# WanqingXia/UR-gym

Measured on AMD Instinct MI355X. Metric: env-steps/sec (whole node), higher is better.
Workload: dtype f64; 1 GPU; UR5DynReach-v1 N=65536 per GPU, random actions U(-1,1), auto-reset, seed 0; envs_total=65536, gather_obs=False, rollout_api=False, gjk_start=bullet

## Files before the change

### ur_gym_amd/csrc/urgym_device.h

```cpp
#pragma once
#include <stdint.h>
#if defined(URGYM_HOST_HARNESS)
#include <cmath>
#define __device__
#define __forceinline__ inline
#define URGYM_LDS
static inline uint32_t __umulhi(uint32_t a, uint32_t b) { return (uint32_t)(((uint64_t)a * b) >> 32); }
using std::fma; using std::sqrt; using std::fabs; using std::fmin; using std::fmax; using std::acos; using std::asin; using std::atan2;
#else
#include <hip/hip_runtime.h>
#define URGYM_LDS __attribute__((address_space(3)))
#endif
#include "urgym_philox.h"

namespace urgym {

struct D3 {
  double x, y, z;
};
__device__ __forceinline__ D3 d3(double x, double y, double z) { return D3{x, y, z}; }
__device__ __forceinline__ D3 operator+(D3 a, D3 b) { return d3(a.x + b.x, a.y + b.y, a.z + b.z); }
__device__ __forceinline__ D3 operator-(D3 a, D3 b) { return d3(a.x - b.x, a.y - b.y, a.z - b.z); }
__device__ __forceinline__ D3 operator-(D3 a) { return d3(-a.x, -a.y, -a.z); }
__device__ __forceinline__ D3 operator*(D3 a, double s) { return d3(a.x * s, a.y * s, a.z * s); }
// ... 253 lines not shown
  if (d3_ >= 0.0 && d4 <= d3_) { mask = 2; return b; }
  double vc = d1 * d4 - d3_ * d2;
  if (vc <= 0.0 && d1 >= 0.0 && d3_ <= 0.0) { mask = 3; return a + ab * (d1 / (d1 - d3_)); }
  double d5 = -dot(ab, c), d6 = -dot(ac, c);
  if (d6 >= 0.0 && d5 <= d6) { mask = 4; return c; }
  double vb = d5 * d2 - d1 * d6;
  if (vb <= 0.0 && d2 >= 0.0 && d6 <= 0.0) { mask = 5; return a + ac * (d2 / (d2 - d6)); }
  double va = d3_ * d6 - d5 * d4;
  if (va <= 0.0 && (d4 - d3_) >= 0.0 && (d5 - d6) >= 0.0) {
    mask = 6;
    return b + (c - b) * ((d4 - d3_) / ((d4 - d3_) + (d5 - d6)));
  }
  double den = 1.0 / (va + vb + vc);
  mask = 7;
  return a + ab * (vb * den) + ac * (vc * den);
}

enum { GJK_PENETRATING = 1, GJK_ITERCAP = 2, GJK_SEPARATED = 4, GJK_CLOSE = 8  };

constexpr int GJK_SLOT_DOUBLES = 24;
__device__ __forceinline__ D3 ldw(XRef T, int i) { return d3(T.at(12 + 3 * i), T.at(13 + 3 * i), T.at(14 + 3 * i)); }
__device__ __forceinline__ void stw(XRef T, int i, D3 w) { T.set(12 + 3 * i, w.x); T.set(13 + 3 * i, w.y); T.set(14 + 3 * i, w.z); }

struct GjkRun {
  D3 v;
  double sq;
  int n;
  int iter;
  int info;
  double core;
  bool done;
};
__device__ __forceinline__ void gjk_begin(GjkRun& r, D3 v0) {
  r.v = v0;
  r.sq = 1.0e300;
  r.n = 0;
  r.iter = 0;
  r.info = 0;
  r.core = 0.0;
  r.done = false;
}
__device__ __forceinline__ void gjk_finish(GjkRun& r, bool check_simplex, bool separated) {
  const double REL_ERROR2 = 1.0e-12;
  const double l2 = len2(r.v);
  r.done = true;
  if (!check_simplex || l2 < REL_ERROR2) {
    if (!(r.info & GJK_ITERCAP)) r.info |= GJK_PENETRATING;
    r.core = 0.0;
    return;
  }
  if (separated) r.info |= GJK_SEPARATED;
  r.core = sqrt(l2);
}
__device__ __forceinline__ void gjk_iterate(GjkRun& r, const HullMap& g, const ShapeDesc& A, XRef T, const ShapeDesc& B, double max_d,
                                            double verdict_d = 0.0) {
  const double REL_ERROR2 = 1.0e-12;
  const double EPS = 2.220446049250313e-16;
  const D3 W0 = ldw(T, 0), W1 = ldw(T, 1), W2 = ldw(T, 2);
  D3 w;
  {
    X3 TX;
#pragma unroll
    for (int k = 0; k < 9; k++) TX.r[k] = T.at(k);
    TX.t = d3(T.at(9), T.at(10), T.at(11));
    const D3 dA = rotT(TX, -r.v);
    int rec = 0;
    if (A.type == SH_HULL) rec = g.cell[A.hull * DIRMAP_CELLS + dirmap_cell(dA)];
    const D3 q = support_local(g, B, r.v);
    const D3 sA = (A.type == SH_HULL) ? hull_support_from(g, rec, dA) : support_local(g, A, dA);
    const D3 p = apply(TX, sA);
    w = p - q;
  }
  int fin = 0;
  const double delta = dot(r.v, w);
  if (delta > 0.0 && delta * delta > r.sq * (max_d * max_d)) fin = 1 | 4;
  if (fin == 0) {
    const bool in = (((int)(r.n > 0) & (int)(len2(W0 - w) <= 1e-12)) | ((int)(r.n > 1) & (int)(len2(W1 - w) <= 1e-12)) |
                     ((int)(r.n > 2) & (int)(len2(W2 - w) <= 1e-12))) != 0;
    const double f0 = r.sq - delta, f1 = r.sq * REL_ERROR2;
    if (in || f0 <= f1) fin = 1;
  }
  if (fin == 0) {
    stw(T, r.n, w);
    int n = r.n + 1;
    D3 nv = d3(0, 0, 0);
    bool valid = true;
    int used = 15;
    bool reduce = true;
    if (n == 1) {
      nv = w;
      reduce = false;
    } else if (n == 2) {
      D3 s0 = W0;
      D3 e = w - s0;
      double t = -dot(e, s0);
      used = 3;
      if (t > 0.0) {
        double ee = dot(e, e);
        if (t < ee) t /= ee;
        else { t = 1.0; used = 2; }
      } else {
        t = 0.0;
        used = 1;
      }
      nv = s0 + e * t;
    } else {
      const bool tetra = (n == 4);
      auto face_vertices = [](int f, int& ia, int& ib, int& ic, int& io) {
        ia = (f == 3) ? 1 : 0;
        ib = (f == 0) ? 1 : ((f == 1) ? 2 : 3);
        ic = (f == 0) ? 2 : ((f == 1) ? 3 : ((f == 2) ? 1 : 2));
        io = (f == 0) ? 3 : ((f == 1) ? 1 : ((f == 2) ? 2 : 0));
      };
      int todo = 1;
      bool degen = false;
      if (tetra) {
        todo = 0;
        auto plane = [&](D3 a, D3 b, D3 c, D3 o, int bit) {
          const D3 nrm = cross(b - a, c - a);
          const double signp = -dot(a, nrm), signd = dot(o - a, nrm);
          if (signd * signd < (1.0e-8 * 1.0e-8)) degen = true;
// ... 6 lines not shown
      }
      double best = 1.0e300;
      used = -1;
#pragma unroll 1
      while (todo) {
        const int f = __builtin_ctz((unsigned)todo);
        todo &= todo - 1;
        int ia, ib, ic, io;
        face_vertices(f, ia, ib, ic, io);
        const D3 a = ldw(T, ia), b = ldw(T, ib), c = ldw(T, ic);
        int m3;
        const D3 pt = tri_closest(a, b, c, m3);
        const double l = len2(pt);
        if (used < 0 || l < best) {
          best = l;
          nv = pt;
          used = ((m3 & 1) ? (1 << ia) : 0) | ((m3 & 2) ? (1 << ib) : 0) | ((m3 & 4) ? (1 << ic) : 0);
        }
      }
      if (degen) {
        valid = false;
        reduce = false;
      } else if (used < 0) {
        nv = d3(0, 0, 0);
        reduce = false;
      }
    }
    if (reduce) {
      if (n >= 4 && !(used & 8)) { n--; }
      if (n >= 3 && !(used & 4)) { n--; stw(T, 2, ldw(T, n)); }
      if (n >= 2 && !(used & 2)) { n--; stw(T, 1, ldw(T, n)); }
      if (n >= 1 && !(used & 1)) { n--; stw(T, 0, ldw(T, n)); }
    }
    r.n = n;
    if (!valid) fin = 1;
    else {
      const double nsq = len2(nv);
      if (nsq < REL_ERROR2) { r.v = nv; fin = 1; }
      else if (nsq <= verdict_d * verdict_d) { r.v = nv; r.info |= GJK_CLOSE; fin = 1; }
      else {
        const double prev = r.sq;
        r.sq = nsq;
        if (prev - nsq <= EPS * prev) fin = 1;
        else {
          r.v = nv;
          if (r.iter++ > 1000) { r.info |= GJK_ITERCAP; fin = 3; }
          else if (n == 4) fin = 3;
        }
      }
    }
  }
  if (fin) gjk_finish(r, !(fin & 2), (fin & 4) != 0);
}


constexpr int EPA_MAX_VERTS = 48, EPA_MAX_FACES = 128;
constexpr int EPA_FACE_GROUPS = EPA_MAX_FACES / 64;
constexpr double EPA_TOL = 1.0e-9, EPA_CAP_RESIDUAL = 1.0e-5;
#if !defined(URGYM_HOST_HARNESS)
struct EpaWs {
  URGYM_LDS double* base;
  int stride;
  __device__ __forceinline__ URGYM_LDS double* at(int r, int c) const { return base + r * stride + c; }
  __device__ __forceinline__ D3 point(int v) const {
    const int r = 3 * (v / 63), c = 1 + v % 63;
    return d3(*at(r, c), *at(r + 1, c), *at(r + 2, c));
  }
  __device__ __forceinline__ void set_point(int v, D3 p) const {
    const int r = 3 * (v / 63), c = 1 + v % 63;
    *at(r, c) = p.x; *at(r + 1, c) = p.y; *at(r + 2, c) = p.z;
  }
  __device__ __forceinline__ URGYM_LDS int* face_word(int f) const {
    return f < 126 ? (URGYM_LDS int*)at(6, 1) + f : (URGYM_LDS int*)at(7, 1) + (f - 126);
  }
  __device__ __forceinline__ URGYM_LDS unsigned short* rim(int c) const { return (URGYM_LDS unsigned short*)at(8 + c / 252, 1) + c % 252; }
  __device__ __forceinline__ URGYM_LDS unsigned char* free_slot(int r) const { return (URGYM_LDS unsigned char*)at(11, 1) + r; }
  __device__ __forceinline__ URGYM_LDS double* plane(int f, int k) const { return at(12 + 4 * (f >> 6) + k, f & 63); }
};
__device__ __forceinline__ void epa_wave_sync() {
  __builtin_amdgcn_fence(__ATOMIC_ACQ_REL, "wavefront");
  __builtin_amdgcn_wave_barrier();
}
__device__ __forceinline__ bool epa_plane(D3 pi, D3 pj, D3 pk, D3& n, double& d) {
  const D3 c = cross(pj - pi, pk - pi);
  const double l2 = len2(c);
  if (l2 > 1e-40) {
    n = c * (1.0 / sqrt(l2));
    d = dot(n, pi);
    return true;
  }
  n = d3(0, 0, 0);
  d = 1e300;
  return false;
}
__device__ inline double epa_wave(const HullMap& g, const ShapeDesc& A, const ShapeDesc& B, EpaWs ws, int lane, bool& capped) {
  const XRef T{ws.base, ws.stride};
  auto supp = [&](D3 n) -> D3 { return apply(T, support_local(g, A, rotT(T, n))) - support_local(g, B, -n); };
  const double t = 0.5773502691896258;
  {
    const D3 p0 = supp(d3(t, t, t)), p1 = supp(d3(t, -t, -t)), p2 = supp(d3(-t, t, -t)), p3 = supp(d3(-t, -t, t));
    if (lane == 0) { ws.set_point(0, p0); ws.set_point(1, p1); ws.set_point(2, p2); ws.set_point(3, p3); }
#pragma unroll
    for (int gi = 0; gi < EPA_FACE_GROUPS; gi++) *ws.face_word(lane + 64 * gi) = 0;
    epa_wave_sync();
    if (lane < 4) {
      int i = lane == 3 ? 1 : 0, j = lane == 0 ? 1 : (lane == 1 ? 3 : (lane == 2 ? 2 : 3)), k = lane == 0 ? 2 : (lane == 1 ? 1 : (lane == 2 ? 3 : 2));
// ... 132 lines not shown
```

### ur_gym_amd/csrc/urgym_hip.hip

```cpp
#include <hip/hip_runtime.h>
#include <stdint.h>
#include <stdio.h>
#include <string.h>
#include <math.h>
#include <new>
#include <vector>

#include "../../include/urgym.h"
#include "../../data/ur5e_model.h"
#include "urgym_device.h"
#include "urgym_launch_plan.h"
#include "urgym_actor.h"
#include "urgym_critic.h"
#include "urgym_pack_map.h"
#include "urgym_weights.h"
#include "urgym_replay.h"
#include "urgym_tables_host.h"

using namespace urgym;


namespace {

constexpr int WAVES = 4;
constexpr int THREADS = GROUP * WAVES;
constexpr uint32_t NO_ITEM = 0xFFFFFFFFu;
constexpr int REFILL_MIN = 16;
constexpr int RESIDENT = 3;
constexpr int SC_ROWS = 19;
constexpr int PAIR_TABLE = 0, PAIR_TRACK = 5, PAIR_SELF = 10;
__host__ __device__ constexpr int self_pair_bit(int la, int lb) {
  return PAIR_SELF + (la == 1 ? 0 : (la == 2 ? 4 : 7)) + (lb - (la + 2));
}

enum { MODE_STEP = 0, MODE_RESET = 1, MODE_REFRESH = 2, MODE_PREFETCH = 3 };
enum { Q_TABLE = 0, Q_TRACK = 1, Q_SELF = 2 };

constexpr double M_HULL = 0.001, M_PRIM = 0.001;
constexpr double CYL_R = 0.05, CYL_H = 0.4, M_CYL = M_PRIM;
constexpr double TABLE_CX = 0.5, TABLE_CY = 0.0, TABLE_CZ = -0.58, TABLE_HX = 0.55, TABLE_HY = 0.9, TABLE_HZ = 0.46;
constexpr double M_TABLE = M_PRIM;
constexpr double TRACK_CX = 0.0, TRACK_CY = 0.0, TRACK_CZ = -0.06, TRACK_HX = 0.1, TRACK_HY = 0.55, TRACK_HZ = 0.06;
constexpr double M_TRACK = M_PRIM;
constexpr double TARGET_BOX_H = 0.025, M_TARGET_BOX = M_PRIM, TARGET_SPHERE_R = 0.02;

struct DevTables {
  double joint_rot[6][9];
  double joint_xyz[6][3];
  double capsule[6][7];
};
__constant__ DevTables c_tab;

constexpr int REC_FIELDS = 36;
enum { REC_GOAL = 0, REC_START = 6, REC_END = 12, REC_VEL = 18, REC_QUAT = 24, REC_LD = 28, REC_DP = 33 };

struct KParams {
  urgym_config cfg;
  urgym_buffers buf;
  HullMap graph;
  int obs_dim, goal_dim;
  uint32_t seed_lo, seed_hi;
  int pp;
  int copy_final;
  int envs;
  int big_blocks;
  int envs_tail;
  double* rec_d;
  int32_t* rec_i;
  int2* rlist;
  int* rcount;
  int rcap;
  double* ld_scratch;
  double* sc_scratch;
  int* rzero;
  int* rzero2;
  int fallback_on;
  int prefetch;
  int inline_ori;
  float neutral_ach[6];
};
__device__ __forceinline__ double& REC(const KParams& P, int slot, int f, int n) {
  return P.rec_d[((size_t)slot * REC_FIELDS + f) * P.cfg.num_envs + n];
}
__device__ __forceinline__ int32_t& RECI(const KParams& P, int slot, int j, int n) {
  return P.rec_i[((size_t)slot * 2 + j) * P.cfg.num_envs + n];
}

__device__ __forceinline__ double& SOA(double* base, int f, int n, int N) { return base[(size_t)f * N + n]; }

__device__ __forceinline__ long long sortable(double x) {
  const long long k = __double_as_longlong(x);
  return k ^ ((k >> 63) & 0x7FFFFFFFFFFFFFFFLL);
}
__device__ __forceinline__ double unsortable(long long k) { return __longlong_as_double(k ^ ((k >> 63) & 0x7FFFFFFFFFFFFFFFLL)); }

__device__ __forceinline__ ShapeDesc hull_desc(int link ) {
  ShapeDesc s;
  s.type = SH_HULL; s.hull = link - 1; s.hx = s.hy = s.hz = 0.0;
  return s;
}
__device__ __forceinline__ ShapeDesc cyl_desc() {
  ShapeDesc s;
  s.type = SH_CYLZ; s.hull = 0;
  s.hx = s.hy = CYL_R - M_CYL; s.hz = 0.5 * CYL_H - M_CYL;
  return s;
}
__device__ __forceinline__ ShapeDesc box_desc(double hx, double hy, double hz, double margin) {
  ShapeDesc s;
  s.type = SH_BOX; s.hull = 0;
  s.hx = hx - margin; s.hy = hy - margin; s.hz = hz - margin;
  return s;
}
__device__ __forceinline__ ShapeDesc point_desc() {
  ShapeDesc s;
  s.type = SH_POINT; s.hull = 0; s.hx = s.hy = s.hz = 0.0;
  return s;
}

__device__ __forceinline__ void fk_joint(X3& T, int k, double s, double c) {
  const double* F = c_tab.joint_rot[k];
  const double* o = c_tab.joint_xyz[k];
  T.t = T.t + rot(T, d3(o[0], o[1], o[2]));
  double g[9];
#pragma unroll
  for (int i = 0; i < 3; i++) {
    g[i * 3 + 0] = F[i * 3 + 0] * c + F[i * 3 + 1] * s;
    g[i * 3 + 1] = F[i * 3 + 1] * c - F[i * 3 + 0] * s;
    g[i * 3 + 2] = F[i * 3 + 2];
  }
  double r[9];
#pragma unroll
// ... 458 lines not shown
          if (seg_box_lower_bound(b0, b1, TABLE_CX, TABLE_CY, TABLE_CZ, TABLE_HX, TABLE_HY, TABLE_HZ) - rb <= lim) pairs |= 1u << (PAIR_TABLE + link - 2);
          if (seg_box_lower_bound(b0, b1, TRACK_CX, TRACK_CY, TRACK_CZ, TRACK_HX, TRACK_HY, TRACK_HZ) - rb <= lim) pairs |= 1u << (PAIR_TRACK + link - 2);
        }
#pragma unroll
        for (int A = 1; A <= 3; A++) {
          if (A <= link - 2) {
            if (segseg_dist(a0[A - 1], a1[A - 1], b0, b1) - c_tab.capsule[A - 1][6] - rb <= lim + M_HULL) pairs |= 1u << self_pair_bit(A, link);
          }
        }
      }
      if (MODE == MODE_STEP) {
        double er, ep, ey;
        rpy_from_quat(rot_to_quat(T.r), er, ep, ey);
        float* orow = B.observation + (size_t)n * OD;
        orow[0] = (float)T.t.x; orow[1] = (float)T.t.y; orow[2] = (float)T.t.z;
        orow[3] = (float)er; orow[4] = (float)ep; orow[5] = (float)ey;
        atomicOr(&s_flags[e], EE_BIT);
      }
    }
    s_pairs[e] = pairs;
    if (pairs) atomicAdd(&s_pending, __popc(pairs));
  }
  if (MODE == MODE_STEP) {
    if (wv >= WAVES - G && lane == 0) __hip_atomic_fetch_add(&s_p1done, 1, __ATOMIC_RELEASE, __HIP_MEMORY_SCOPE_WORKGROUP);
  } else {
    __syncthreads();
  }

  if (!(MODE == MODE_STEP && !HAS_OBST && !cfg.check_collision)) {
    D3 v0 = d3(0, 1, 0);
    int kind = 3, e = 0, lb = 2, la = 1;
    auto shape_a = [&]() -> ShapeDesc { return hull_desc(kind == Q_SELF ? la : lb); };
    auto shape_b = [&]() -> ShapeDesc {
      ShapeDesc s;
      s.type = (kind == 3) ? SH_CYLZ : ((kind == Q_SELF) ? SH_HULL : SH_BOX);
      s.hull = lb - 1;
      const bool tbl = (kind == Q_TABLE);
      s.hx = (kind == 3) ? (CYL_R - M_CYL) : (tbl ? (TABLE_HX - M_TABLE) : (TRACK_HX - M_TRACK));
      s.hy = (kind == 3) ? (CYL_R - M_CYL) : (tbl ? (TABLE_HY - M_TABLE) : (TRACK_HY - M_TRACK));
      s.hz = (kind == 3) ? (0.5 * CYL_H - M_CYL) : (tbl ? (TABLE_HZ - M_TABLE) : (TRACK_HZ - M_TRACK));
      return s;
    };
    bool exact = false;
    const bool guided = cfg.gjk_start == URGYM_GJK_START_GUIDED;
    auto capsule_mid = [&](int link, const X3& TX) -> D3 {
      const double* c = c_tab.capsule[link - 1];
      return apply(TX, d3(0.5 * (c[0] + c[3]), 0.5 * (c[1] + c[4]), 0.5 * (c[2] + c[5])));
    };
    auto guided_axis = [&](D3 mid, D3 centre) -> D3 {
      const D3 d = mid - centre;
      const double n2 = dot(d, d);
      return n2 > 1e-12 ? d * (1.0 / sqrt(n2)) : d3(0, 1, 0);
    };
    bool p1_ok = false;
    auto setup = [&](uint32_t item) -> bool {
      e = item & 255;
      kind = (item >> 8) & 3;
      exact = ((item >> 16) & 1) != 0;
      lb = (item >> 10) & 7;
      la = (item >> 13) & 7;
      if (e >= E || lb < 1 || lb > 6 || (kind == Q_SELF && (la < 1 || la > 6))) return false;
      const int n = s_env[e];
      if (n < 0) return false;
      const bool cached = (MODE == MODE_STEP) && p1_ok;
      if (MODE == MODE_STEP && !cached) {
        bool finite = true;
        for (int k = 0; k < 6; k++) finite = finite && (fabs(joint_of_step<MODE>(P, actions, n, k)) < 1.0e6);
        if (!finite) return false;
      }
      X3 T = identity_x3(), TA = identity_x3();
#pragma unroll 1
      for (int k = 0; k < lb; k++) {
        double sn, cs;
        if (cached) { sn = SOA(P.sc_scratch, 2 * k, n, N); cs = SOA(P.sc_scratch, 2 * k + 1, n, N); }
        else sincos(LDS_Q ? s_q[k][e] : joint_of_step<MODE>(P, actions, n, k), &sn, &cs);
        fk_joint(T, k, sn, cs);
        if (k + 1 == la) TA = T;
      }
      if (kind == 3) {
        X3 To;
        if (LDS_STATE) {
          quat_to_rot(Q4{s_obst[3][e], s_obst[4][e], s_obst[5][e], s_obst[6][e]}, To.r);
          To.t = d3(s_obst[0][e], s_obst[1][e], s_obst[2][e]);
        } else if (cached) {
          quat_to_rot(Q4{SOA(P.sc_scratch, 15, n, N), SOA(P.sc_scratch, 16, n, N), SOA(P.sc_scratch, 17, n, N), SOA(P.sc_scratch, 18, n, N)}, To.r);
          To.t = d3(SOA(P.sc_scratch, 12, n, N), SOA(P.sc_scratch, 13, n, N), SOA(P.sc_scratch, 14, n, N));
        } else {
          double op[3];
          Q4 oqs;
          obstacle_of_step<KIND>(P, n, op, oqs);
          quat_to_rot(oqs, To.r);
          To.t = d3(op[0], op[1], op[2]);
        }
        store(pose_slot, rel(To, T));
        v0 = rotT(To, guided ? guided_axis(capsule_mid(lb, T), To.t) : d3(0, 1, 0));
      } else if (kind == Q_SELF) {
        store(pose_slot, rel(T, TA));
        v0 = rotT(T, guided ? guided_axis(capsule_mid(la, TA), capsule_mid(lb, T)) : d3(0, 1, 0));
      } else {
        const bool tbl = (kind == Q_TABLE);
        const D3 centre = d3(tbl ? TABLE_CX : TRACK_CX, tbl ? TABLE_CY : TRACK_CY, tbl ? TABLE_CZ : TRACK_CZ);
        v0 = guided ? guided_axis(capsule_mid(lb, T), centre) : d3(0, 1, 0);
        T.t = T.t - centre;
        store(pose_slot, T);
      }
      return true;
    };
    auto claim_pair = [&]() -> uint32_t {
      int pe = tid % E;
#pragma unroll 1
      for (int trip = 0; trip < 2 * ME; trip++, pe = (pe + 1 == E ? 0 : pe + 1)) {
        uint32_t m = s_pairs[pe];
        while (m) {
          const int b = __ffs((int)m) - 1;
          const uint32_t old = atomicAnd(&s_pairs[pe], ~(1u << b));
          if (old & (1u << b)) {
            if (b < PAIR_TRACK) return (uint32_t)pe | (Q_TABLE << 8) | ((uint32_t)(b - PAIR_TABLE + 2) << 10);
            if (b < PAIR_SELF) return (uint32_t)pe | (Q_TRACK << 8) | ((uint32_t)(b - PAIR_TRACK + 2) << 10);
            const int i = b - PAIR_SELF;
            const int la = i < 4 ? 1 : (i < 7 ? 2 : 3);
            const int l2 = i < 4 ? 3 + i : (i < 7 ? i : i - 2);
            return (uint32_t)pe | (Q_SELF << 8) | ((uint32_t)l2 << 10) | ((uint32_t)la << 13);
          }
          m = old & ~(1u << b);
        }
      }
      return NO_ITEM;
    };
    auto margin_sum = [&]() -> double {
      return M_HULL + ((kind == 3) ? M_CYL : ((kind == Q_SELF) ? M_HULL : ((kind == Q_TABLE) ? M_TABLE : M_TRACK)));
    };
    const int n_tickets = HAS_OBST ? (workbench ? 15 : 5) * E : 0;
    auto ticket_item = [&](int t) -> uint32_t {
      const int body = t / (5 * E), r = t - body * 5 * E;
      const int tl = r / E, te = r - tl * E, link = 2 + tl;
      if (body == 0) return (uint32_t)te | (3u << 8) | ((uint32_t)link << 10);
      return (uint32_t)te | ((uint32_t)(body == 1 ? Q_TABLE : Q_TRACK) << 8) | ((uint32_t)link << 10) | (1u << 16);
    };

    GjkRun run;
    bool busy = false;
    if (MODE == MODE_STEP) p1_ok = __hip_atomic_load(&s_p1done, __ATOMIC_ACQUIRE, __HIP_MEMORY_SCOPE_WORKGROUP) >= G;
    if (tid < n_tickets) {
      busy = setup(ticket_item(tid));
      if (busy) gjk_begin(run, v0);
    }
    for (;;) {
      if (busy) {
        if (MODE == MODE_STEP) {
          const URGYM_LDS double* row = (const URGYM_LDS double*)(URGYM_LDS void*)&L.s_kind[kind | ((int)exact << 2)][0];
          ShapeDesc sb;
          sb.type = (kind == 3) ? SH_CYLZ : ((kind == Q_SELF) ? SH_HULL : SH_BOX);
          sb.hull = lb - 1;
          sb.hx = row[0]; sb.hy = row[1]; sb.hz = row[2];
          gjk_iterate(run, P.graph, shape_a(), pose_slot, sb, row[3], row[4]);
        } else {
          const bool wants_distance = (kind == 3 || exact);
          const double verdict_d = wants_distance ? 0.0 : margin_sum() + cfg.collision_margin;
          gjk_iterate(run, P.graph, shape_a(), pose_slot, shape_b(), wants_distance ? margin_sum() + 0.02 + 5.0 : verdict_d, verdict_d);
        }
        if (run.done) {
          const double msum = margin_sum();
          if (kind == 3 || exact) {
            double dist = run.core - msum;
            if (run.info & GJK_PENETRATING) {
              dist = -msum;
              const int body = (kind == 3) ? 0 : (kind == Q_TABLE ? 1 : 2);
              atomicOr(&s_flags[e], URGYM_STATUS_PENETRATION | (need_epa ? (1 << (EPA_SHIFT + 5 * body + (lb - 2))) : 0));
            }
            if (run.info & GJK_ITERCAP) atomicOr(&s_flags[e], URGYM_STATUS_GJK_ITER);
            if (workbench) atomicMin(reinterpret_cast<long long*>(dist_cell(lb - 2, e)), sortable(dist));
            else *dist_cell(lb - 2, e) = dist;
          } else {
            const bool hit = (run.info & (GJK_PENETRATING | GJK_CLOSE)) || (!(run.info & GJK_SEPARATED) && (run.core - msum) <= cfg.collision_margin);
            if (hit) atomicOr(&s_flags[e], COLL_BIT);
          }
          busy = false;
        }
      }
      typedef int pool_words __attribute__((ext_vector_type(4)));
      const pool_words pool = *(volatile URGYM_LDS pool_words*)(URGYM_LDS void*)&s_ticket;
      __builtin_amdgcn_fence(__ATOMIC_ACQUIRE, "workgroup");
      const bool more_tickets = pool.x < n_tickets;
      const bool p1_published = (MODE != MODE_STEP) || pool.z >= G;
      const bool more_pairs = pool.y > 0;
      if (MODE == MODE_STEP) p1_ok = p1_published;
      const int idle_lanes = __popcll(__ballot(!busy));
      if (!busy && (idle_lanes >= REFILL_MIN || idle_lanes == 64)) {
        uint32_t item = NO_ITEM;
        if (more_tickets) {
          const int t = atomicAdd(&s_ticket, 1);
          if (t < n_tickets) item = ticket_item(t);
        } else if (more_pairs) {
          if (atomicSub(&s_pending, 1) > 0) item = claim_pair();
        }
        if (item != NO_ITEM) {
          busy = setup(item);
          if (busy) gjk_begin(run, v0);
        }
      }
      if (__ballot(busy) == 0ull && !more_tickets && !more_pairs && p1_published) break;
    }
    auto epa_pass = [&]() -> bool {
      const EpaWs ws{(URGYM_LDS double*)&s_pose[0][0] + GROUP * wv, THREADS};
      bool armed = false;
#pragma unroll 1
      for (int g = 0; g < G; g++) {
        const int sl = g * GROUP + lane;
        const int marks = (sl < E) ? ((__hip_atomic_load(&s_flags[sl], __ATOMIC_RELAXED, __HIP_MEMORY_SCOPE_WORKGROUP) & EPA_MASK) >> EPA_SHIFT) : 0;
        unsigned long long envs_marked = __ballot(marks != 0);
#pragma unroll 1
        while (envs_marked) {
          const int el = __builtin_ctzll(envs_marked);
          envs_marked &= envs_marked - 1ull;
          const int ee = g * GROUP + el;
          int me = __shfl(marks, el);
#pragma unroll 1
          while (me) {
            const int b = __builtin_ctz((unsigned)me);
            me &= me - 1;
            int mine = 0;
            if (lane == 0) mine = (atomicAnd(&s_flags[ee], ~(1 << (EPA_SHIFT + b))) >> (EPA_SHIFT + b)) & 1;
            if (!__shfl(mine, 0)) continue;
            if (!armed) {
              pose_slot.p = ws.base;
              if (MODE == MODE_STEP) p1_ok = true;
              armed = true;
            }
            const int body = b / 5, link = 2 + b - 5 * body;
            const uint32_t item = (uint32_t)ee | ((uint32_t)(body == 0 ? 3 : (body == 1 ? Q_TABLE : Q_TRACK)) << 8) | ((uint32_t)link << 10) |
                                  ((body ? 1u : 0u) << 16);
            if (!setup(item)) continue;
            epa_wave_sync();
            bool capped;
            const double depth = epa_wave(P.graph, shape_a(), shape_b(), ws, lane, capped);
            if (lane == 0) {
              const double dist = -(depth + margin_sum());
              if (workbench) atomicMin(reinterpret_cast<long long*>(dist_cell(lb - 2, e)), sortable(dist));
              else *dist_cell(lb - 2, e) = dist;
              if (capped) atomicOr(&s_flags[e], URGYM_STATUS_GJK_ITER);
            }
          }
        }
      }
      if (armed) pose_slot.p = (URGYM_LDS double*)&s_pose[0][0] + tid;
      return armed;
    };
    if (HAS_OBST && WITH_EPA) {
      if (lane == 0) __hip_atomic_fetch_add(&s_left, 1, __ATOMIC_RELEASE, __HIP_MEMORY_SCOPE_WORKGROUP);
#pragma unroll 1
      for (;;) {
        const int left = __hip_atomic_load(&s_left, __ATOMIC_ACQUIRE, __HIP_MEMORY_SCOPE_WORKGROUP);
        const bool served = epa_pass();
        if (!served && left >= WAVES) break;
        if (!served) __builtin_amdgcn_s_sleep(16);
      }
    }
    __syncthreads();
  }

  const int pe = (wv - (WAVES - G)) * GROUP + lane;
  if (wv >= WAVES - G && pe < E && s_env[pe] != -1) {
    const int n = s_env[pe] >= 0 ? s_env[pe] : -2 - s_env[pe];
    double q[6];
    for (int i = 0; i < 6; i++) q[i] = LDS_Q ? s_q[i][pe] : joint_of_step<MODE>(P, actions, n, i);
    const bool ee_ready = (MODE == MODE_STEP) && (s_flags[pe] & EE_BIT);
    X3 TE = identity_x3();
    if (!ee_ready) {
      if (KIND == URGYM_ENV_ORI) {
        double sn[6], cs[6];
#pragma unroll
        for (int k = 0; k < 6; k++) sincos(q[k], &sn[k], &cs[k]);
#pragma unroll
        for (int k = 0; k < 6; k++) fk_joint(TE, k, sn[k], cs[k]);
      } else {
#pragma unroll 1
        for (int k = 0; k < 6; k++) {
          double sn, cs;
          sincos(q[k], &sn, &cs);
          fk_joint(TE, k, sn, cs);
        }
      }
    }
    double opos[3] = {0, 0, 0};
    Q4 oq{0, 0, 0, 1};
// ... 509 lines not shown
  c->near_threshold = 0.2;
  c->collision_margin = 0.01;
  c->target_clearance = 0.1;
  c->min_travel = 1.0;
  c->dyn_time_duration = 2.0;
  const double neutral[6] = {0.0, -1.5708, 0.0, -1.5708, 0.0, 0.0};
  for (int i = 0; i < 6; i++) c->neutral_q[i] = neutral[i];
  if (env_kind == URGYM_ENV_ORI) {
    c->w_distance = -70; c->w_orientation = -30;
    const double gl[3] = {0.3, -0.5, 0.0}, gh[3] = {0.75, 0.5, 0.2};
    for (int i = 0; i < 3; i++) { c->goal_low[i] = gl[i]; c->goal_high[i] = gh[i]; }
  } else if (env_kind == URGYM_ENV_OBS) {
    c->w_distance = -100; c->w_orientation = 0;
    const double gl[3] = {0.3, -0.5, -0.1}, gh[3] = {0.75, 0.5, 0.2}, ol[3] = {0.5, -0.5, 0.25}, oh[3] = {1.0, 0.5, 0.55};
    for (int i = 0; i < 3; i++) { c->goal_low[i] = gl[i]; c->goal_high[i] = gh[i]; c->obst_low[i] = ol[i]; c->obst_high[i] = oh[i]; }
    for (int i = 0; i < 5; i++) c->w_link[i] = 100.0;
  } else {
    c->w_distance = -70; c->w_orientation = -30;
    const double gl[3] = {0.4, -0.5, 0.0}, gh[3] = {0.75, 0.5, 0.2}, ol[3] = {0.5, -0.8, 0.25}, oh[3] = {1.2, 0.8, 0.75};
    const double sgl[3] = {0.3, -0.5, 0.0}, sgh[3] = {0.75, 0.5, 0.2}, sol[3] = {0.5, -0.5, 0.25}, soh[3] = {1.0, 0.5, 0.55};
    const bool sta = env_kind == URGYM_ENV_STA;
    for (int i = 0; i < 3; i++) {
      c->goal_low[i] = sta ? sgl[i] : gl[i]; c->goal_high[i] = sta ? sgh[i] : gh[i];
      c->obst_low[i] = sta ? sol[i] : ol[i]; c->obst_high[i] = sta ? soh[i] : oh[i];
    }
    const double lw[5] = {8, 2.4, 1.2, 1.2, 0.2};
    double sum = 0;
    for (int i = 0; i < 5; i++) sum += lw[i];
    for (int i = 0; i < 5; i++) c->w_link[i] = lw[i] / sum * 50;
  }
}

KParams make_params(Handle* h, int copy_final) {
  KParams P{};
  P.cfg = h->cfg;
  P.buf = h->buf;
  P.graph.recs = h->d_recs;
  P.graph.cell = h->d_cell;
  P.obs_dim = h->obs_dim;
  P.goal_dim = h->goal_dim;
  P.seed_lo = (uint32_t)h->seed;
  P.seed_hi = (uint32_t)(h->seed >> 32);
  P.pp = h->pp;
  P.copy_final = copy_final;
  P.envs = h->plan.step_envs;
  P.big_blocks = h->plan.big_blocks;
  P.envs_tail = h->plan.tail_envs;
  P.rec_d = h->d_rec;
  P.rec_i = h->d_reci;
  P.ld_scratch = h->d_ld_scratch;
  P.sc_scratch = h->d_sc_scratch;
  P.fallback_on = 1;
  P.inline_ori = h->plan.inline_ori ? 1 : 0;
  for (int i = 0; i < 6; i++) P.neutral_ach[i] = h->neutral_ach[i];
  return P;
}

template <int MODE>
void launch_mode(Handle* h, KParams P, const float* actions, hipStream_t s, int envs = 0, long items = -1) {
  long blocks = h->plan.step_blocks;
  if (MODE != MODE_STEP) {
    const int cap = (MODE == MODE_PREFETCH) ? PREFETCH_MAX_ENVS : MAX_ENVS;
    P.envs = envs < 1 ? 1 : (envs > cap ? cap : envs);
    if (items < 0) items = h->cfg.num_envs;
    blocks = (items + P.envs - 1) / P.envs;
  }
  hipLaunchKernelGGL(h->k.mode[MODE], dim3((unsigned)blocks), dim3(THREADS), 0, s, P, actions);
}

void launch_fused(Handle* h, KParams Ps, KParams Pr, const float* actions, hipStream_t s) {
  Pr.envs = PREFETCH_MAX_ENVS;
  const int sb = h->plan.step_blocks;
  const long grid = sb + refill_blocks(h->plan, h->steps_since_full_reset, h->cfg.max_episode_steps);
  hipLaunchKernelGGL(h->k.fused, dim3((unsigned)grid), dim3(THREADS), 0, s, Ps, Pr, actions, sb);
}

int time_begin(Handle* h, int kind, hipStream_t s) {
  if (!h->timing || h->ev_used >= 65536) return -1;
  if (kind == 0 && (h->timing_tick++ % h->timing_every) != 0) return -1;
  if (h->ev_used + 2 > h->ev.size()) {
    for (int i = 0; i < 2; i++) {
      hipEvent_t e;
      if (hipEventCreate(&e) != hipSuccess) return -1;
      h->ev.push_back(e);
    }
    h->ev_kind.push_back(kind);
  }
  h->ev_kind[h->ev_used / 2] = kind;
  hipEventRecord(h->ev[h->ev_used], s);
  return (int)h->ev_used;
}
void time_end(Handle* h, int slot, hipStream_t s) {
  if (slot < 0) return;
  hipEventRecord(h->ev[slot + 1], s);
  h->ev_used = slot + 2;
}

int enter_bound(Handle* h) {
  if (!h) return fail(nullptr, URGYM_ERR_ARG, "null handle");
  if (!h->bound) return fail(h, URGYM_ERR_STATE, "urgym_bind() has not been called");
  HIP_TRY(h, hipSetDevice(h->device));
  return URGYM_OK;
}

void release(Handle* h) {
  for (void* p : {(void*)h->d_ld_scratch, (void*)h->d_sc_scratch, (void*)h->d_recs, (void*)h->d_cell, (void*)h->d_rec,
// ... 928 lines not shown
```

### ur_gym_amd/csrc/urgym_launch_plan.h

```cpp
#pragma once
#include <limits.h>
#include <stdio.h>
#include <stdlib.h>

#include <algorithm>

#include "../../include/urgym.h"

namespace urgym {

constexpr int GROUP = 64;
constexpr int PREFETCH_MAX_ENVS = 32;
constexpr int MAX_ENVS = 64;
constexpr int STEP_MAX_ENVS = 128;

struct Tuning {
  int step_envs, reset_envs, refill_blocks;
  int tiers = -1, tier_envs = 0, tier_blocks = 0, tier_tail = 0;
  bool prefetch;
  bool verbose;
};

inline Tuning read_tuning() {
  auto number = [](const char* name, int lo, int hi) {
    const char* v = getenv(name);
    const int x = v ? atoi(v) : 0;
    return x < lo || x > hi ? 0 : x;
  };
  Tuning t;
  t.step_envs = number("URGYM_STEP_ENVS", 1, STEP_MAX_ENVS);
  t.reset_envs = number("URGYM_RESET_ENVS", 1, MAX_ENVS);
  t.refill_blocks = number("URGYM_REFILL_BLOCKS", 1, INT_MAX);
  const char* pf = getenv("URGYM_PREFETCH");
  t.prefetch = !pf || atoi(pf) != 0;
  t.verbose = getenv("URGYM_VERBOSE") != nullptr;
  if (const char* v = getenv("URGYM_STEP_TIERS")) {
    int e1 = 0, b = 0, e2 = 0;
    if (sscanf(v, "%d,%d,%d", &e1, &b, &e2) == 3 && e1 >= 1 && e1 <= STEP_MAX_ENVS && e2 >= 1 && e2 <= STEP_MAX_ENVS && b >= 1)
      t.tiers = 1, t.tier_envs = e1, t.tier_blocks = b, t.tier_tail = e2;
    else if (atoi(v) == 0)
      t.tiers = 0;
  }
  return t;
}

struct LaunchPlan {
  int num_envs = 0;
  int step_envs = GROUP, big_blocks = 0, tail_envs = 0, step_blocks = 0;
  int reset_envs = 4;
  bool prefetch = false;
  bool fused = false;
  bool inline_ori = false;
  static constexpr int setup_cache = 1;
  int rl_cap[4] = {0, 0, 0, 0};
  int refill_blocks = 0;
};

inline LaunchPlan plan_paths(int env_kind, int num_envs, bool auto_reset, const Tuning& t) {
  LaunchPlan p;
  p.num_envs = num_envs;
  p.prefetch = env_kind != URGYM_ENV_ORI && t.prefetch;
  p.fused = p.prefetch && auto_reset;
  p.inline_ori = env_kind == URGYM_ENV_ORI && t.prefetch;
  p.refill_blocks = t.refill_blocks;
  if (p.prefetch) {
    p.rl_cap[0] = p.rl_cap[1] = p.rl_cap[2] = num_envs;
    p.rl_cap[3] = 2 * num_envs;
  }
  return p;
}

inline void plan_grids(LaunchPlan& p, int cus, int per_cu, const Tuning& t) {
  const long n = p.num_envs;
  long slots = (long)cus * per_cu;
  if (p.fused) {
    const long refill = n / 1600;
    slots -= refill < slots / 8 ? refill : slots / 8;
  }
  const long rounds = (n + slots * STEP_MAX_ENVS - 1) / (slots * STEP_MAX_ENVS);
  long envs = (n + slots * rounds - 1) / (slots * rounds);
  if (envs < 8) envs = 8;
  if (envs < GROUP) envs = (envs + 7) / 8 * 8;
  if (envs > STEP_MAX_ENVS) envs = STEP_MAX_ENVS;
  p.step_envs = (int)envs;
  if (rounds == 1 && per_cu == 3 && slots > 2L * cus) {
    const long big = 2L * cus, rest = slots - big;
    const long e1 = (10 * n + (10 * big + 7 * rest) - 1) / (10 * big + 7 * rest);
    if (e1 >= 64 && e1 <= STEP_MAX_ENVS && n > big * e1) {
      const long e2 = (n - big * e1 + rest - 1) / rest;
      p.step_envs = (int)e1; p.big_blocks = (int)big; p.tail_envs = (int)(e2 < 1 ? 1 : e2);
    }
  }
  while (p.reset_envs < GROUP && n / 100 > (long)p.reset_envs * (cus + cus / 4)) p.reset_envs *= 2;
  if (t.step_envs) { p.step_envs = t.step_envs; p.big_blocks = p.tail_envs = 0; }
  if (t.tiers == 1) { p.step_envs = t.tier_envs; p.big_blocks = t.tier_blocks; p.tail_envs = t.tier_tail; }
  if (t.tiers == 0) { p.step_envs = (int)envs; p.big_blocks = p.tail_envs = 0; }
  if (t.reset_envs) p.reset_envs = t.reset_envs;
  if (p.big_blocks > 0 && (long)p.big_blocks * p.step_envs >= n) p.big_blocks = p.tail_envs = 0;
  if (p.big_blocks > 0)
    p.step_blocks = (int)(p.big_blocks + (n - (long)p.big_blocks * p.step_envs + p.tail_envs - 1) / p.tail_envs);
  else
    p.step_blocks = (int)((n + p.step_envs - 1) / p.step_envs);
}

inline bool step_geometry_ok(const LaunchPlan& p) {
  const long n = p.num_envs, blocks = p.step_blocks;
  if (p.step_envs < 1 || p.step_envs > STEP_MAX_ENVS || blocks < 1) return false;
  if (p.tail_envs == 0) return (blocks - 1) * p.step_envs < n && blocks * p.step_envs >= n;
  if (p.tail_envs < 1 || p.tail_envs > STEP_MAX_ENVS || p.big_blocks < 1 || p.big_blocks >= blocks) return false;
  const long covered_before_last = (long)p.big_blocks * p.step_envs + (blocks - p.big_blocks - 1) * p.tail_envs;
  return covered_before_last < n && covered_before_last + p.tail_envs >= n;
}

inline long refill_blocks(const LaunchPlan& p, long steps_since_full_reset, int max_episode_steps) {
  const long full = ((long)p.rl_cap[0] + PREFETCH_MAX_ENVS - 1) / PREFETCH_MAX_ENVS;
  if (p.refill_blocks > 0) return std::min<long>(p.refill_blocks, full);
  const long s = steps_since_full_reset, m = max_episode_steps;
// ... 6 lines not shown
```

Measured before the change: 320.9 million env-steps/s.

## Specialize collision tickets for cylinder obstacle pairs with wave-uniform fast path

Makes the GJK iteration generic over the support function of shape B. In step mode with obstacles, the initial tickets are set up as link-vs-cylinder pairs through a compile-time specialised setup that can read cached sin/cos values. When the whole wave is doing cylinder pairs, it uses constant margins and a hard-coded cylinder support instead of reading per-kind rows from LDS. The aim is to cut setup and LDS-load overhead and keep lanes uniform. The change adds code size and register pressure and depends on a new env toggle that is on by default.

```diff
diff --git a/ur_gym_amd/csrc/urgym_device.h b/ur_gym_amd/csrc/urgym_device.h
--- a/ur_gym_amd/csrc/urgym_device.h
+++ b/ur_gym_amd/csrc/urgym_device.h
@@ -329,8 +329,9 @@
   if (separated) r.info |= GJK_SEPARATED;
   r.core = sqrt(l2);
 }
-__device__ __forceinline__ void gjk_iterate(GjkRun& r, const HullMap& g, const ShapeDesc& A, XRef T, const ShapeDesc& B, double max_d,
-                                            double verdict_d = 0.0) {
+template <class SupportB>
+__device__ __forceinline__ void gjk_iterate_with(GjkRun& r, const HullMap& g, const ShapeDesc& A, XRef T, const SupportB& support_b, double max_d,
+                                                 double verdict_d = 0.0) {
   const double REL_ERROR2 = 1.0e-12;
   const double EPS = 2.220446049250313e-16;
   const D3 W0 = ldw(T, 0), W1 = ldw(T, 1), W2 = ldw(T, 2);
@@ -343,7 +344,7 @@
     const D3 dA = rotT(TX, -r.v);
     int rec = 0;
     if (A.type == SH_HULL) rec = g.cell[A.hull * DIRMAP_CELLS + dirmap_cell(dA)];
-    const D3 q = support_local(g, B, r.v);
+    const D3 q = support_b(r.v);
     const D3 sA = (A.type == SH_HULL) ? hull_support_from(g, rec, dA) : support_local(g, A, dA);
     const D3 p = apply(TX, sA);
     w = p - q;
@@ -456,6 +457,10 @@
   }
   if (fin) gjk_finish(r, !(fin & 2), (fin & 4) != 0);
 }
+__device__ __forceinline__ void gjk_iterate(GjkRun& r, const HullMap& g, const ShapeDesc& A, XRef T, const ShapeDesc& B, double max_d,
+                                            double verdict_d = 0.0) {
+  gjk_iterate_with(r, g, A, T, [&](D3 d) -> D3 { return support_local(g, B, d); }, max_d, verdict_d);
+}
 
 
 constexpr int EPA_MAX_VERTS = 48, EPA_MAX_FACES = 128;
diff --git a/ur_gym_amd/csrc/urgym_hip.hip b/ur_gym_amd/csrc/urgym_hip.hip
--- a/ur_gym_amd/csrc/urgym_hip.hip
+++ b/ur_gym_amd/csrc/urgym_hip.hip
@@ -4,6 +4,7 @@
 #include <string.h>
 #include <math.h>
 #include <new>
+#include <type_traits>
 #include <vector>
 
 #include "../../include/urgym.h"
@@ -77,6 +78,7 @@
   int fallback_on;
   int prefetch;
   int inline_ori;
+  int ticket_body;
   float neutral_ach[6];
 };
 __device__ __forceinline__ double& REC(const KParams& P, int slot, int f, int n) {
@@ -642,16 +644,17 @@
       return n2 > 1e-12 ? d * (1.0 / sqrt(n2)) : d3(0, 1, 0);
     };
     bool p1_ok = false;
-    auto setup = [&](uint32_t item) -> bool {
+    auto setup_as = [&](uint32_t item, auto cyl, auto from_cache) -> bool {
+      constexpr bool CYL = decltype(cyl)::value, FROM_CACHE = decltype(from_cache)::value;
       e = item & 255;
-      kind = (item >> 8) & 3;
-      exact = ((item >> 16) & 1) != 0;
+      kind = CYL ? 3 : (item >> 8) & 3;
+      exact = CYL ? false : ((item >> 16) & 1) != 0;
       lb = (item >> 10) & 7;
-      la = (item >> 13) & 7;
-      if (e >= E || lb < 1 || lb > 6 || (kind == Q_SELF && (la < 1 || la > 6))) return false;
+      la = CYL ? 0 : (item >> 13) & 7;
+      if (e >= E || lb < 1 || lb > 6 || (!CYL && kind == Q_SELF && (la < 1 || la > 6))) return false;
       const int n = s_env[e];
       if (n < 0) return false;
-      const bool cached = (MODE == MODE_STEP) && p1_ok;
+      const bool cached = (MODE == MODE_STEP) && (FROM_CACHE || p1_ok);
       if (MODE == MODE_STEP && !cached) {
         bool finite = true;
         for (int k = 0; k < 6; k++) finite = finite && (fabs(joint_of_step<MODE>(P, actions, n, k)) < 1.0e6);
@@ -664,13 +667,14 @@
         if (cached) { sn = SOA(P.sc_scratch, 2 * k, n, N); cs = SOA(P.sc_scratch, 2 * k + 1, n, N); }
         else sincos(LDS_Q ? s_q[k][e] : joint_of_step<MODE>(P, actions, n, k), &sn, &cs);
         fk_joint(T, k, sn, cs);
-        if (k + 1 == la) TA = T;
-      }
-      if (kind == 3) {
+        if (!CYL && k + 1 == la) TA = T;
+      }
+      if (CYL || kind == 3) {
         X3 To;
         if (LDS_STATE) {
-          quat_to_rot(Q4{s_obst[3][e], s_obst[4][e], s_obst[5][e], s_obst[6][e]}, To.r);
-          To.t = d3(s_obst[0][e], s_obst[1][e], s_obst[2][e]);
+          constexpr int R = LDS_STATE ? 1 : 0;
+          quat_to_rot(Q4{s_obst[3 * R][e], s_obst[4 * R][e], s_obst[5 * R][e], s_obst[6 * R][e]}, To.r);
+          To.t = d3(s_obst[0][e], s_obst[R][e], s_obst[2 * R][e]);
         } else if (cached) {
           quat_to_rot(Q4{SOA(P.sc_scratch, 15, n, N), SOA(P.sc_scratch, 16, n, N), SOA(P.sc_scratch, 17, n, N), SOA(P.sc_scratch, 18, n, N)}, To.r);
           To.t = d3(SOA(P.sc_scratch, 12, n, N), SOA(P.sc_scratch, 13, n, N), SOA(P.sc_scratch, 14, n, N));
@@ -695,6 +699,7 @@
       }
       return true;
     };
+    auto setup = [&](uint32_t item) -> bool { return setup_as(item, std::false_type{}, std::false_type{}); };
     auto claim_pair = [&]() -> uint32_t {
       int pe = tid % E;
 #pragma unroll 1
@@ -727,15 +732,75 @@
       return (uint32_t)te | ((uint32_t)(body == 1 ? Q_TABLE : Q_TRACK) << 8) | ((uint32_t)link << 10) | (1u << 16);
     };
 
+    const bool ticket_body = (MODE == MODE_STEP) && HAS_OBST && P.ticket_body != 0;
+    auto cyl_ticket_item = [&](int t) -> uint32_t {
+      const int tl = t / E, te = t - tl * E;
+      return (uint32_t)te | (3u << 8) | ((uint32_t)(2 + tl) << 10);
+    };
+
     GjkRun run;
     bool busy = false;
     if (MODE == MODE_STEP) p1_ok = __hip_atomic_load(&s_p1done, __ATOMIC_ACQUIRE, __HIP_MEMORY_SCOPE_WORKGROUP) >= G;
     if (tid < n_tickets) {
-      busy = setup(ticket_item(tid));
+      busy = (ticket_body && !workbench) ? setup_as(cyl_ticket_item(tid), std::true_type{}, std::false_type{}) : setup(ticket_item(tid));
       if (busy) gjk_begin(run, v0);
     }
     for (;;) {
-      if (busy) {
+      const bool cyl_trip = ticket_body && __ballot(busy && kind != 3) == 0ull;
+      if (MODE == MODE_STEP && HAS_OBST) {
+        if (busy) {
+          double max_d, verdict_d;
+          if (cyl_trip) {
+            max_d = M_HULL + M_CYL + 0.02 + 5.0; verdict_d = 0.0;
+          } else {
+            const URGYM_LDS double* row = (const URGYM_LDS double*)(URGYM_LDS void*)&L.s_kind[kind | ((int)exact << 2)][0];
+            max_d = row[3]; verdict_d = row[4];
+          }
+          gjk_iterate_with(run, P.graph, shape_a(), pose_slot, [&](D3 d) -> D3 {
+            ShapeDesc sb;
+            if (cyl_trip) {
+              sb.type = SH_CYLZ; sb.hull = 0;
+              sb.hx = sb.hy = CYL_R - M_CYL; sb.hz = 0.5 * CYL_H - M_CYL;
+              return support_local(P.graph, sb, d);
+            }
+            const URGYM_LDS double* row = (const URGYM_LDS double*)(URGYM_LDS void*)&L.s_kind[kind | ((int)exact << 2)][0];
+            sb.type = (kind == 3) ? SH_CYLZ : ((kind == Q_SELF) ? SH_HULL : SH_BOX);
+            sb.hull = lb - 1;
+            sb.hx = row[0]; sb.hy = row[1]; sb.hz = row[2];
+            return support_local(P.graph, sb, d);
+          }, max_d, verdict_d);
+          if (run.done) {
+            if (cyl_trip) {
+              constexpr double msum = M_HULL + M_CYL;
+              double dist = run.core - msum;
+              if (run.info & GJK_PENETRATING) {
+                dist = -msum;
+                atomicOr(&s_flags[e], URGYM_STATUS_PENETRATION | (need_epa ? (1 << (EPA_SHIFT + (lb - 2))) : 0));
+              }
+              if (run.info & GJK_ITERCAP) atomicOr(&s_flags[e], URGYM_STATUS_GJK_ITER);
+              if (workbench) atomicMin(reinterpret_cast<long long*>(dist_cell(lb - 2, e)), sortable(dist));
+              else *dist_cell(lb - 2, e) = dist;
+            } else {
+              const double msum = margin_sum();
+              if (kind == 3 || exact) {
+                double dist = run.core - msum;
+                if (run.info & GJK_PENETRATING) {
+                  dist = -msum;
+                  const int body = (kind == 3) ? 0 : (kind == Q_TABLE ? 1 : 2);
+                  atomicOr(&s_flags[e], URGYM_STATUS_PENETRATION | (need_epa ? (1 << (EPA_SHIFT + 5 * body + (lb - 2))) : 0));
+                }
+                if (run.info & GJK_ITERCAP) atomicOr(&s_flags[e], URGYM_STATUS_GJK_ITER);
+                if (workbench) atomicMin(reinterpret_cast<long long*>(dist_cell(lb - 2, e)), sortable(dist));
+                else *dist_cell(lb - 2, e) = dist;
+              } else {
+                const bool hit = (run.info & (GJK_PENETRATING | GJK_CLOSE)) || (!(run.info & GJK_SEPARATED) && (run.core - msum) <= cfg.collision_margin);
+                if (hit) atomicOr(&s_flags[e], COLL_BIT);
+              }
+            }
+            busy = false;
+          }
+        }
+      } else if (busy) {
         if (MODE == MODE_STEP) {
           const URGYM_LDS double* row = (const URGYM_LDS double*)(URGYM_LDS void*)&L.s_kind[kind | ((int)exact << 2)][0];
           ShapeDesc sb;
@@ -777,14 +842,15 @@
       const int idle_lanes = __popcll(__ballot(!busy));
       if (!busy && (idle_lanes >= REFILL_MIN || idle_lanes == 64)) {
         uint32_t item = NO_ITEM;
+        const bool cyl_draw = ticket_body && !workbench && more_tickets && p1_published;
         if (more_tickets) {
           const int t = atomicAdd(&s_ticket, 1);
-          if (t < n_tickets) item = ticket_item(t);
+          if (t < n_tickets) item = cyl_draw ? cyl_ticket_item(t) : ticket_item(t);
         } else if (more_pairs) {
           if (atomicSub(&s_pending, 1) > 0) item = claim_pair();
         }
         if (item != NO_ITEM) {
-          busy = setup(item);
+          busy = cyl_draw ? setup_as(item, std::true_type{}, std::true_type{}) : setup(item);
           if (busy) gjk_begin(run, v0);
         }
       }
@@ -1435,6 +1501,7 @@
   P.sc_scratch = h->d_sc_scratch;
   P.fallback_on = 1;
   P.inline_ori = h->plan.inline_ori ? 1 : 0;
+  P.ticket_body = h->plan.ticket_body ? 1 : 0;
   for (int i = 0; i < 6; i++) P.neutral_ach[i] = h->neutral_ach[i];
   return P;
 }
diff --git a/ur_gym_amd/csrc/urgym_launch_plan.h b/ur_gym_amd/csrc/urgym_launch_plan.h
--- a/ur_gym_amd/csrc/urgym_launch_plan.h
+++ b/ur_gym_amd/csrc/urgym_launch_plan.h
@@ -19,6 +19,7 @@
   int tiers = -1, tier_envs = 0, tier_blocks = 0, tier_tail = 0;
   bool prefetch;
   bool verbose;
+  bool ticket_body = true;
 };
 
 inline Tuning read_tuning() {
@@ -34,6 +35,8 @@
   const char* pf = getenv("URGYM_PREFETCH");
   t.prefetch = !pf || atoi(pf) != 0;
   t.verbose = getenv("URGYM_VERBOSE") != nullptr;
+  const char* tb = getenv("URGYM_TICKET_BODY");
+  t.ticket_body = !tb || atoi(tb) != 0;
   if (const char* v = getenv("URGYM_STEP_TIERS")) {
     int e1 = 0, b = 0, e2 = 0;
     if (sscanf(v, "%d,%d,%d", &e1, &b, &e2) == 3 && e1 >= 1 && e1 <= STEP_MAX_ENVS && e2 >= 1 && e2 <= STEP_MAX_ENVS && b >= 1)
@@ -51,6 +54,7 @@
   bool prefetch = false;
   bool fused = false;
   bool inline_ori = false;
+  bool ticket_body = true;
   static constexpr int setup_cache = 1;
   int rl_cap[4] = {0, 0, 0, 0};
   int refill_blocks = 0;
@@ -63,6 +67,7 @@
   p.fused = p.prefetch && auto_reset;
   p.inline_ori = env_kind == URGYM_ENV_ORI && t.prefetch;
   p.refill_blocks = t.refill_blocks;
+  p.ticket_body = t.ticket_body;
   if (p.prefetch) {
     p.rl_cap[0] = p.rl_cap[1] = p.rl_cap[2] = num_envs;
     p.rl_cap[3] = 2 * num_envs;
```

Measured after the change: 322.3 million env-steps/s (median of 6 runs). Within noise of the previous version (+0.4%).

## Restructure GJK work loop to iterate until enough lanes idle before refilling

Applied to the files above, without the earlier changes.

The GJK iteration body becomes an inlined lambda that runs repeatedly until at least REFILL_MIN lanes are idle, so the shared ticket/pool state is read and the refill logic runs less often per GJK step. Setup is specialised at compile time so items claimed after phase-1 publication always use the cached sin/cos path, dropping the finiteness check and sincos recompute. The exit condition re-checks s_p1done and s_pending and drains busy lanes in a final loop. In exchange, lanes sit idle longer before refilling, and the idle==64 refill path is gone, which could shift load balance or termination behaviour.

```diff
diff --git a/ur_gym_amd/csrc/urgym_hip.hip b/ur_gym_amd/csrc/urgym_hip.hip
--- a/ur_gym_amd/csrc/urgym_hip.hip
+++ b/ur_gym_amd/csrc/urgym_hip.hip
@@ -4,6 +4,7 @@
 #include <string.h>
 #include <math.h>
 #include <new>
+#include <type_traits>
 #include <vector>
 
 #include "../../include/urgym.h"
@@ -641,8 +642,8 @@
       const double n2 = dot(d, d);
       return n2 > 1e-12 ? d * (1.0 / sqrt(n2)) : d3(0, 1, 0);
     };
-    bool p1_ok = false;
-    auto setup = [&](uint32_t item) -> bool {
+    bool p1_ok = (MODE != MODE_STEP);
+    auto setup = [&](uint32_t item, auto after_p1) -> bool {
       e = item & 255;
       kind = (item >> 8) & 3;
       exact = ((item >> 16) & 1) != 0;
@@ -651,7 +652,7 @@
       if (e >= E || lb < 1 || lb > 6 || (kind == Q_SELF && (la < 1 || la > 6))) return false;
       const int n = s_env[e];
       if (n < 0) return false;
-      const bool cached = (MODE == MODE_STEP) && p1_ok;
+      const bool cached = (MODE == MODE_STEP) && (decltype(after_p1)::value || p1_ok);
       if (MODE == MODE_STEP && !cached) {
         bool finite = true;
         for (int k = 0; k < 6; k++) finite = finite && (fabs(joint_of_step<MODE>(P, actions, n, k)) < 1.0e6);
@@ -731,10 +732,10 @@
     bool busy = false;
     if (MODE == MODE_STEP) p1_ok = __hip_atomic_load(&s_p1done, __ATOMIC_ACQUIRE, __HIP_MEMORY_SCOPE_WORKGROUP) >= G;
     if (tid < n_tickets) {
-      busy = setup(ticket_item(tid));
+      busy = setup(ticket_item(tid), std::false_type{});
       if (busy) gjk_begin(run, v0);
     }
-    for (;;) {
+    auto trip = [&]() __attribute__((always_inline)) {
       if (busy) {
         if (MODE == MODE_STEP) {
           const URGYM_LDS double* row = (const URGYM_LDS double*)(URGYM_LDS void*)&L.s_kind[kind | ((int)exact << 2)][0];
@@ -767,6 +768,9 @@
           busy = false;
         }
       }
+    };
+    for (;;) {
+      do trip(); while (__popcll(__ballot(!busy)) < REFILL_MIN);
       typedef int pool_words __attribute__((ext_vector_type(4)));
       const pool_words pool = *(volatile URGYM_LDS pool_words*)(URGYM_LDS void*)&s_ticket;
       __builtin_amdgcn_fence(__ATOMIC_ACQUIRE, "workgroup");
@@ -774,8 +778,7 @@
       const bool p1_published = (MODE != MODE_STEP) || pool.z >= G;
       const bool more_pairs = pool.y > 0;
       if (MODE == MODE_STEP) p1_ok = p1_published;
-      const int idle_lanes = __popcll(__ballot(!busy));
-      if (!busy && (idle_lanes >= REFILL_MIN || idle_lanes == 64)) {
+      if (!busy && p1_ok) {
         uint32_t item = NO_ITEM;
         if (more_tickets) {
           const int t = atomicAdd(&s_ticket, 1);
@@ -784,11 +787,22 @@
           if (atomicSub(&s_pending, 1) > 0) item = claim_pair();
         }
         if (item != NO_ITEM) {
-          busy = setup(item);
+          busy = setup(item, std::true_type{});
           if (busy) gjk_begin(run, v0);
         }
       }
-      if (__ballot(busy) == 0ull && !more_tickets && !more_pairs && p1_published) break;
+      if (!more_tickets && !more_pairs && p1_published) {
+        bool dry = true;
+        if (MODE == MODE_STEP) {
+          const int done = __hip_atomic_load(&s_p1done, __ATOMIC_ACQUIRE, __HIP_MEMORY_SCOPE_WORKGROUP);
+          const int pending = __hip_atomic_load(&s_pending, __ATOMIC_RELAXED, __HIP_MEMORY_SCOPE_WORKGROUP);
+          dry = done >= G && pending <= 0;
+        }
+        if (dry) {
+          while (__ballot(busy) != 0ull) trip();
+          break;
+        }
+      }
     }
     auto epa_pass = [&]() -> bool {
       const EpaWs ws{(URGYM_LDS double*)&s_pose[0][0] + GROUP * wv, THREADS};
@@ -819,7 +833,7 @@
             const int body = b / 5, link = 2 + b - 5 * body;
             const uint32_t item = (uint32_t)ee | ((uint32_t)(body == 0 ? 3 : (body == 1 ? Q_TABLE : Q_TRACK)) << 8) | ((uint32_t)link << 10) |
                                   ((body ? 1u : 0u) << 16);
-            if (!setup(item)) continue;
+            if (!setup(item, std::true_type{})) continue;
             epa_wave_sync();
             bool capped;
             const double depth = epa_wave(P.graph, shape_a(), shape_b(), ws, lane, capped);
```

After: 321.6 million env-steps/s before, 331.8 million env-steps/s after (median of 6 runs). +3.2%, better.
